# yemam3/SAC-RCBF

Measured on AMD Instinct MI355X. Metric: safe env steps/sec (dynamics+CBF-QP) at batch 65536, 1/2/4/8 MI355X, higher is better.
Workload: dtype f32 rows / f64 QP / f64 env

## Files before the change

### sac-rcbf_amd/csrc/rcbf_device.hpp

```cpp
#pragma once

#include <hip/hip_runtime.h>
#include <stdint.h>

#include "rcbf_hip.h"

namespace rcbf {

constexpr double kInf = __builtin_huge_val();


#ifdef RCBF_STUDY_QP_STAMPS
__device__ __forceinline__ void qp_stamp(int j) {
    __builtin_amdgcn_sched_barrier(0);
    unsigned long long t;
    asm volatile("s_memtime %0\n\ts_waitcnt lgkmcnt(0)" : "=s"(t)::"memory");
    __builtin_amdgcn_sched_barrier(0);
    if ((threadIdx.x & 63) == 0 && rcbf_qp_stamp_buf)
        rcbf_qp_stamp_buf[((int64_t)blockIdx.x * 4 + (threadIdx.x >> 6)) * 16 + j] = t;
}
__device__ __forceinline__ void qp_count(int j, bool f) {
    const unsigned long long n = __popcll(__ballot(f));
    if ((threadIdx.x & 63) == 0 && rcbf_qp_stamp_buf)
        rcbf_qp_stamp_buf[((int64_t)blockIdx.x * 4 + (threadIdx.x >> 6)) * 16 + j] = n;
// ... 1679 lines not shown
    double c, s;
    sincos(xs[2], &s, &c);
    double px = xs[0] + lp * c, py = xs[1] + lp * s;
    double g00 = c, g01 = -s * lp, g10 = s, g11 = c * lp;
    double mpx = mu[0] + lp * (-s) * mu[2], mpy = mu[1] + lp * c * mu[2];
    double spx = sig[0] + lp * (-s) * sig[2], spy = sig[1] + lp * c * sig[2];
    const double r2 = (1.2 * prm.hazards_radius) * (1.2 * prm.hazards_radius);
#pragma unroll
    for (int j = 0; j < K; ++j) {
        double dx = px - prm.hazards_xy[2 * j], dy = py - prm.hazards_xy[2 * j + 1];
        double hs = 0.5 * ((dx * dx + dy * dy) - r2);
        double a0 = dx * g00 + dy * g10, a1 = dx * g01 + dy * g11;
        G[j][0] = -a0;
        G[j][1] = -a1;
        G[j][2] = -1.0;
        h[j] = ((g * (hs * hs * hs) + (dx * mpx + dy * mpy)) + (a0 * u[0] + a1 * u[1])) -
               kd * (fabs(dx) * spx + fabs(dy) * spy);
    }
#pragma unroll
    for (int c2 = 0; c2 < 2; ++c2) {
        const int r0 = K + 2 * c2;
#pragma unroll
        for (int k = 0; k < 3; ++k) {
            G[r0][k] = (k == c2) ? 1.0 : 0.0;
            G[r0 + 1][k] = (k == c2) ? -1.0 : 0.0;
        }
        h[r0] = prm.u_max[c2] - u[c2];
        h[r0 + 1] = -prm.u_min[c2] + u[c2];
    }
}

struct CarsStepOut {
    float reward;
    double reward_d;
    double cost;
    bool done;
};

__device__ __forceinline__ double cars_env_pre(const rcbf_params& prm, double* xs, double& t, int& step,
                                               CarsStepOut& o) {
#pragma clang fp contract(off)
    const double kp = prm.kp, kb = prm.k_brake, dt = 0.02;
    double vdes0 = 30.0 - 10.0 * sin_small(0.2 * t);
    double acc[5];
    acc[0] = kp * (vdes0 - xs[1]);
#pragma unroll
    for (int i = 1; i < 5; ++i) acc[i] = kp * (30.0 - xs[2 * i + 1]);
    double d01 = xs[0] - xs[2], d12 = xs[2] - xs[4], d24 = xs[4] - xs[8];
    acc[1] += (-kb * d01) * (d01 < 6.0 ? 1.0 : 0.0);
    acc[2] += (-kb * d12) * (d12 < 6.0 ? 1.0 : 0.0);
    acc[4] += (-kb * d24) * (d24 < 13.0 ? 1.0 : 0.0);
#pragma unroll
    for (int i = 0; i < 5; ++i) acc[i] *= 1.1;
    double v[5];
#pragma unroll
    for (int i = 0; i < 5; ++i) v[i] = xs[2 * i + 1];
#pragma unroll
    for (int i = 0; i < 5; ++i) {
        xs[2 * i] += dt * v[i];
        if (i != 3) xs[2 * i + 1] += dt * acc[i];
    }
    t = t + dt;
    step += 1;
    o.done = step >= 300;
    double cost = 0.0;
    if (xs[4] - xs[6] < 2.99) cost -= 0.1;
    if (xs[6] - xs[8] < 2.99) cost -= 0.1;
    o.cost = cost;
    return acc[3];
}

template <typename A>
__device__ __forceinline__ void cars_env_post(double* xs, double acc3, A action, CarsStepOut& o) {
#pragma clang fp contract(off)
    const double dt = 0.02;
    const double gu = 50.0 * (double)action;
    xs[7] += dt * (acc3 + gu);
    A a2 = action * action;
    A r = (A)(-5.0) * (a2 < (A)0 ? -a2 : a2) / (A)300;
    o.reward = (float)r;
    o.reward_d = (double)r;
}

template <typename A>
__device__ __forceinline__ void cars_env_step(const rcbf_params& prm, double* xs, double& t, int& step, A action,
                                              CarsStepOut& o) {
    const double acc3 = cars_env_pre(prm, xs, t, step, o);
    cars_env_post<A>(xs, acc3, action, o);
}

__device__ __forceinline__ double div_const(double x, double d, double inv_d) {
    double q = x * inv_d;
    double r = fma(-q, d, x);
    return fma(r, inv_d, q);
}

__device__ __forceinline__ void cars_obs(const double* xs, double* o) {
#pragma unroll
    for (int i = 0; i < 5; ++i) {
        o[2 * i] = div_const(xs[2 * i], 100.0, 1.0 / 100.0);
        o[2 * i + 1] = div_const(xs[2 * i + 1], 30.0, 1.0 / 30.0);
    }
}

__device__ __forceinline__ void sincos_add_small(double c, double s, double d, double& c2, double& s2) {
    const double d2 = d * d;
    const double sd =
        d * fma(d2, fma(d2, fma(d2, fma(d2, 1.0 / 362880.0, -1.0 / 5040.0), 1.0 / 120.0), -1.0 / 6.0), 1.0);
    const double cd =
        fma(d2, fma(d2, fma(d2, fma(d2, 1.0 / 40320.0, -1.0 / 720.0), 1.0 / 24.0), -0.5), 1.0);
    c2 = fma(c, cd, -(s * sd));
    s2 = fma(s, cd, c * sd);
}

__device__ __forceinline__ double uni_goal_dist(const double* xs) {
#pragma clang fp contract(off)
    double d0 = 2.5 - xs[0], d1 = 2.5 - xs[1];
    return sqrt(d0 * d0 + d1 * d1);
}

__device__ __forceinline__ void uni_obs_cs(const double* xs, double c, double s, double gd, double* o) {
#pragma clang fp contract(off)
    double r0 = 2.5 - xs[0], r1 = 2.5 - xs[1];
    double v0 = r0 * c + r1 * s;
    double v1 = r0 * (-s) + r1 * c;
    double nrm = sqrt(v0 * v0 + v1 * v1) + 0.001;
    const double rn = rcp64_nz(nrm);
    o[0] = xs[0];
    o[1] = xs[1];
    o[2] = c;
    o[3] = s;
    o[4] = v0 * rn;
    o[5] = v1 * rn;
    o[6] = exp(-gd);
}

__device__ __forceinline__ void uni_obs(const double* xs, double* o) {
#pragma clang fp contract(off)
    double r0 = 2.5 - xs[0], r1 = 2.5 - xs[1];
    double gd = sqrt(r0 * r0 + r1 * r1);
    double c, s;
    sincos(xs[2], &s, &c);
    double v0 = r0 * c + r1 * s;
    double v1 = r0 * (-s) + r1 * c;
    double nrm = sqrt(v0 * v0 + v1 * v1) + 0.001;
    o[0] = xs[0];
    o[1] = xs[1];
    o[2] = c;
    o[3] = s;
    o[4] = v0 / nrm;
    o[5] = v1 / nrm;
    o[6] = exp(-gd);
}

struct UniStepOut {
    double reward;
    double cost;
    bool done;
    bool goal;
    double c, s, gd;
};

template <typename A, int KH = 0>
__device__ __forceinline__ void uni_env_step_cs(const rcbf_params& prm, double* xs, double& last_dist, int& step,
                                                const A* action, double c, double s, UniStepOut& o) {
#pragma clang fp contract(off)
    A a0c = action[0] < (A)(-1) ? (A)(-1) : (action[0] > (A)1 ? (A)1 : action[0]);
    A a1c = action[1] < (A)(-1) ? (A)(-1) : (action[1] > (A)1 ? (A)1 : action[1]);
    double a0 = (double)a0c, a1 = (double)a1c;
    const double dt = 0.02;
    xs[0] += dt * (c * a0);
    xs[1] += dt * (s * a0);
    const double th0 = xs[2];
    xs[2] += dt * a1;
    double c2, s2;
    sincos_add_small(c, s, xs[2] - th0, c2, s2);
    const double k = dt * 0.1;
    xs[0] -= (k * c2) * c2;
    xs[1] -= (k * s2) * c2;
    o.c = c2;
    o.s = s2;
    step += 1;
    double d = uni_goal_dist(xs);
    o.gd = d;
// ... 69 lines not shown
```

### sac-rcbf_amd/csrc/rcbf_safe_step.hpp

```cpp
#pragma once

#include <cstddef>

#include "rcbf_common.hpp"

#ifndef RCBF_KARG_PREFETCH
#define RCBF_KARG_PREFETCH 0
#endif
#ifndef RCBF_TRAJ_OBS_PLAIN
#define RCBF_TRAJ_OBS_PLAIN 0
#endif
#ifndef RCBF_EARLY_STORE
#define RCBF_EARLY_STORE 1
#endif
#ifndef RCBF_FUSED_CARRY
#define RCBF_FUSED_CARRY 1
#endif
#ifndef RCBF_FUSED_CARRY_SOLVE_FIRST
#define RCBF_FUSED_CARRY_SOLVE_FIRST 0
#endif

namespace rcbf {

template <int NL>
__device__ __forceinline__ void prefetch_kernargs() {
#if defined(__HIP_DEVICE_COMPILE__)
    __builtin_amdgcn_sched_barrier(0);
    const uint32_t* ka = (const uint32_t*)__builtin_amdgcn_kernarg_segment_ptr();
    uint32_t acc = 0;
#pragma unroll
    for (int l = 0; l < NL; ++l) acc ^= ka[16 * l];
    asm volatile("" ::"s"(acc));
    __builtin_amdgcn_sched_barrier(0);
#endif
}

template <int MODE>
__device__ __forceinline__ void load_state(const double* x, int64_t B, int64_t i, double* xs) {
    constexpr int NS = Dims<MODE, 1>::NS;
#pragma unroll
    for (int p = 0; p < NS / 2; ++p) {
        double2 v = ld_in2(&x[2 * (p * B + i)]);
        xs[2 * p] = v.x;
        xs[2 * p + 1] = v.y;
    }
    if constexpr (NS % 2) xs[NS - 1] = ld_in(&x[(NS - 1) * B + i]);
}

template <int MODE, typename XP = double*>
__device__ __forceinline__ void store_state(XP x, int64_t B, int64_t i, const double* xs) {
    constexpr int NS = Dims<MODE, 1>::NS;
#pragma unroll
    for (int p = 0; p < NS / 2; ++p) st_out2d(&x[2 * (p * B + i)], xs[2 * p], xs[2 * p + 1]);
    if constexpr (NS % 2) st_out(&x[(NS - 1) * B + i], xs[NS - 1]);
}

template <int MODE, bool WT = false, typename OP = float*>
__device__ __forceinline__ void store_obs32(OP obs, int64_t i, const double* xs,
                                            const double* obs_cache = nullptr) {
    constexpr int NO = Dims<MODE, 1>::NO;
    double o[NO];
    if constexpr (MODE == RCBF_MODE_UNICYCLE) {
        if (obs_cache && obs_cache[3] != 0.0)
            uni_obs_cs(xs, obs_cache[0], obs_cache[1], obs_cache[2], o);
        else
            env_obs<MODE>(xs, o);
    } else {
        env_obs<MODE>(xs, o);
    }
    if constexpr (MODE == RCBF_MODE_SIMULATED_CARS) {
        const OP ov = obs + i * NO;
#pragma unroll
        for (int k = 0; k < NO / 2; ++k) {
            if constexpr (WT) {
                const float pr[2] = {(float)o[2 * k], (float)o[2 * k + 1]};
                uint64_t w;
                __builtin_memcpy(&w, pr, 8);
                st_wt(reinterpret_cast<uint64_t*>(ov + 2 * k), w);
            } else {
                st_out2(ov + 2 * k, (float)o[2 * k], (float)o[2 * k + 1]);
            }
        }
    } else {
#pragma unroll
        for (int k = 0; k < NO; ++k) st_any<WT>(&obs[i * NO + k], (float)o[k]);
    }
}

template <int MODE, bool WT = false, bool SC1 = WT || MODE == RCBF_MODE_SIMULATED_CARS, typename OP = float*,
          bool PLAIN_ST = false, bool WHOLE = false>
__device__ __forceinline__ void store_obs_chunks(OP obs, int64_t base, const float* lds_wave, int lane) {
    constexpr int NO = Dims<MODE, 1>::NO;
    __builtin_amdgcn_wave_barrier();
    constexpr int CH = NO * 16;
    const float4* src = reinterpret_cast<const float4*>(lds_wave);
    const OP dst = obs + base * NO;
    constexpr int NJ = (CH + 63) / 64;
    float4 chunk[NJ];
    if constexpr (WHOLE) {
#pragma unroll
        for (int j = 0; j < NJ; ++j) {
            const int c = j * 64 + lane;
            chunk[j] = src[(j < CH / 64 || c < CH) ? c : lane];
        }
#pragma unroll
        for (int j = 0; j < NJ; ++j) asm volatile("" : "+v"(chunk[j].x), "+v"(chunk[j].y), "+v"(chunk[j].z), "+v"(chunk[j].w));
#pragma unroll
        for (int j = 0; j < NJ; ++j) {
            const int c = j * 64 + lane;
            if (j < CH / 64 || c < CH) {
                if constexpr (PLAIN_ST)
                    st_out4_plain(dst + 4 * c, chunk[j]);
                else
                    st_out4<SC1>(dst + 4 * c, chunk[j]);
            }
        }
        return;
    }
#pragma unroll
    for (int j = 0; j < NJ; ++j) {
        const int c = j * 64 + lane;
        if (CH % 64 == 0 || c < CH) chunk[j] = src[c];
    }
#pragma unroll
    for (int j = 0; j < NJ; ++j) {
        const int c = j * 64 + lane;
        if (CH % 64 == 0 || c < CH) {
            if constexpr (PLAIN_ST)
                st_out4_plain(dst + 4 * c, chunk[j]);
            else
                st_out4<SC1>(dst + 4 * c, chunk[j]);
        }
    }
}

template <int MODE, bool WT = false, bool SC1 = WT || MODE == RCBF_MODE_SIMULATED_CARS, typename OP = float*,
          bool PLAIN_ST = false>
__device__ __forceinline__ void store_obs32_staged(OP obs, int64_t i, int64_t B, const double* xs,
                                                   const double* obs_cache, float* lds_wave, int lane) {
    constexpr int NO = Dims<MODE, 1>::NO;
    const int64_t base = i - lane;
#ifdef RCBF_STUDY_EPW
    const bool full = blockDim.x != 64 && (base + 64 <= B) && ((reinterpret_cast<uintptr_t>(obs) & 15) == 0);
#else
    const bool full = (base + 64 <= B) && ((reinterpret_cast<uintptr_t>(obs) & 15) == 0);
#endif
    if (!full) {
        store_obs32<MODE, WT>(obs, i, xs, obs_cache);
        return;
    }
    double o[NO];
    if constexpr (MODE == RCBF_MODE_UNICYCLE) {
        if (obs_cache && obs_cache[3] != 0.0)
            uni_obs_cs(xs, obs_cache[0], obs_cache[1], obs_cache[2], o);
        else
            env_obs<MODE>(xs, o);
    } else {
        env_obs<MODE>(xs, o);
    }
    if constexpr (NO % 2 == 0) {
#pragma unroll
        for (int k = 0; k < NO / 2; ++k)
            *reinterpret_cast<float2*>(&lds_wave[lane * NO + 2 * k]) = make_float2((float)o[2 * k], (float)o[2 * k + 1]);
    } else {
#pragma unroll
        for (int k = 0; k < NO; ++k) lds_wave[lane * NO + k] = (float)o[k];
    }
    store_obs_chunks<MODE, WT, SC1, OP, PLAIN_ST>(obs, base, lds_wave, lane);
}

template <int MODE, typename OP>
__device__ __forceinline__ bool stage_obs32_row(OP obs, int64_t i, int64_t B, const float* o32, float* lds_wave,
                                                int lane) {
    constexpr int NO = Dims<MODE, 1>::NO;
    static_assert(NO % 2 == 0, "8-byte halves of a row");
    const int64_t base = i - lane;
#ifdef RCBF_STUDY_EPW
    const bool full_l = blockDim.x != 64 && (base + 64 <= B) && ((reinterpret_cast<uintptr_t>(obs) & 15) == 0);
#else
    const bool full_l = (base + 64 <= B) && ((reinterpret_cast<uintptr_t>(obs) & 15) == 0);
#endif
    const bool full = __builtin_amdgcn_readfirstlane((int)full_l) != 0;
    if (full) {
#pragma unroll
        for (int k = 0; k < NO / 2; ++k)
            *reinterpret_cast<float2*>(&lds_wave[lane * NO + 2 * k]) = make_float2(o32[2 * k], o32[2 * k + 1]);
    } else {
        const OP ov = obs + i * NO;
#pragma unroll
        for (int k = 0; k < NO / 2; ++k) st_out2(ov + 2 * k, o32[2 * k], o32[2 * k + 1]);
    }
    return full;
}

template <int SOLVER, int MODE, int K, bool ST, bool WT, bool GP = false,
          bool OBS_SC1 = WT || MODE == RCBF_MODE_SIMULATED_CARS, bool OBS_PLAIN = false, int CARRY = 0,
          bool TERM = false>
__device__ __forceinline__ void safe_step_body(
    const rcbf_params& prm, int64_t B, int64_t i, ptr_g<GP, double> __restrict__ x, ptr_g<GP, double> __restrict__ aux,
    ptr_g<GP, int32_t> __restrict__ step, ptr_g<GP, uint32_t> __restrict__ episode,
    ptr_g<GP, float> __restrict__ obs_out, ptr_g<GP, float> __restrict__ u_out, ptr_g<GP, float> __restrict__ reward,
    ptr_g<GP, float> __restrict__ cost, ptr_g<GP, uint8_t> __restrict__ done, ptr_g<GP, uint8_t> __restrict__ goal_met,
    ptr_g<GP, int32_t> __restrict__ status_out, ptr_g<GP, int32_t> fail_flag, int auto_reset,
    uint64_t seed, int64_t off, double* xs, double& a, int& st, const float* us, const float* m, const float* s,
    bool ep_pre, uint32_t ep0, const Stamps<ST>& stamps, float* obs_stage, char* wt_lds, int lane,
    bool* did_reset = nullptr, float* obs_c = nullptr, float (*G_c)[Dims<MODE, K>::N] = nullptr,
    float* h_c = nullptr, const float* u_nx = nullptr, ptr_g<GP, float> term_obs = nullptr) {
    using D = Dims<MODE, K>;
    static_assert(!TERM || (GP && !ST && !WT && SOLVER == RCBF_SOLVER_ACTIVE_SET &&
                            (MODE != RCBF_MODE_SIMULATED_CARS || RCBF_EARLY_STORE)),
                  "the terminal observation: the fused loop only");
    static_assert(CARRY == 0 || (MODE == RCBF_MODE_SIMULATED_CARS && RCBF_EARLY_STORE && !ST && !WT && GP &&
                                 SOLVER == RCBF_SOLVER_ACTIVE_SET && RCBF_FUSED_RAW_ROWS != 0),
                  "the carried observation: the cars fused loop only");
    const int64_t wbase = i - lane;
    const bool wfull = wbase + 64 <= B;
    constexpr int kWtBytes = WT ? 16 * 160 : 16;
    (void)wt_lds;
    (void)wfull;
    (void)kWtBytes;
    float rew, cst;
    bool dn, gm;
    int status;
    float uf[D::NU];
    double oc[4] = {0.0, 0.0, 0.0, 0.0};
    if constexpr (MODE == RCBF_MODE_SIMULATED_CARS && RCBF_EARLY_STORE && !ST) {
        float s32[D::NS];
        if constexpr (CARRY == 0) state_from_env<MODE>(xs, s32);
        if constexpr (CARRY == 1) state_from_obs32<MODE>(obs_c, s32);
        constexpr bool kRowsFirst = SOLVER == RCBF_SOLVER_ACTIVE_SET && RCBF_FUSED_RAW_ROWS != 0;
        LayerState<MODE, K> L;
        if constexpr (CARRY == 2) {
#pragma unroll
            for (int r = 0; r < D::M; ++r) {
                L.h[r] = h_c[r];
#pragma unroll
                for (int k = 0; k < D::N; ++k) L.G[r][k] = G_c[r][k];
            }
        } else if constexpr (kRowsFirst) {
            diff_rows<MODE, K>(prm, s32, us, m, s, L.G, L.h, nullptr);
        }
        constexpr bool kSolveFirst = CARRY == 2 && RCBF_FUSED_CARRY_SOLVE_FIRST != 0;
        if constexpr (kSolveFirst) {
            layer_solve_raw<MODE, K>(prm, us, uf, L);
            __builtin_amdgcn_sched_barrier(0);
        }
        CarsStepOut o;
        const double acc3 = cars_env_pre(prm, xs, a, st, o);
        dn = o.done;
        cst = (float)o.cost;
        gm = false;
        const bool rs = auto_reset && dn;
        if (rs) {
            if constexpr (TERM) {
                double ot[D::NO];
                env_obs<MODE>(xs, ot);
#pragma unroll
                for (int k = 0; k < D::NO; ++k)
                    if (k != 7) st_out(&term_obs[i * D::NO + k], (float)ot[k]);
                oc[0] = xs[7];
            }
            const uint32_t ep = episode ? (ep_pre ? ep0 : episode[i]) + 1u : 0u;
            if (episode) {
                if constexpr (WT)
                    st_wt(&episode[i], ep);
                else
                    episode[i] = ep;
            }
            env_reset_one<MODE>(nullptr, i, seed, off, ep, xs, a, st);
        }
#pragma unroll
        for (int p = 0; p < D::NS / 2; ++p)
            if (p != 3) st_any2d<WT>(&x[2 * (p * B + i)], xs[2 * p], xs[2 * p + 1]);
        if constexpr (WT) {
            using E = WtStage<8, 4>;
            char* const dst[2] = {reinterpret_cast<char*>(aux + wbase), reinterpret_cast<char*>(step + wbase)};
            const uint64_t val[2] = {wt_bits(a), wt_bits(st)};
            E::store(wt_lds, lane, wfull, dst, val);
        } else {
            st_out(&aux[i], a);
            st_out(&step[i], st);
        }
        __builtin_amdgcn_sched_barrier(0);
        if constexpr (kSolveFirst) {
        } else if constexpr (kRowsFirst) {
            layer_solve_raw<MODE, K>(prm, us, uf, L);
        } else {
            layer_forward<SOLVER, MODE, K, false, false, RCBF_FUSED_RAW_ROWS != 0>(prm, s32, us, m, s, uf, L);
        }
        status = L.qp.status;
        const double v3_reset = xs[7];
        if constexpr (TERM) xs[7] = rs ? oc[0] : xs[7];
        cars_env_post<float>(xs, acc3, uf[0], o);
        if constexpr (TERM) {
            if (rs) st_out(&term_obs[i * D::NO + 7], (float)div_const(xs[7], 30.0, 1.0 / 30.0));
        }
        xs[7] = rs ? v3_reset : xs[7];
        rew = o.reward;
        st_any2d<WT>(&x[2 * (3 * B + i)], xs[6], xs[7]);
    } else {
        if constexpr (TERM) {
            static_assert(MODE == RCBF_MODE_UNICYCLE, "the cars loop takes the early-store path");
            safe_step_one<SOLVER, MODE, K, ST, WT>(prm, i, xs, a, st, episode, us, m, s, uf, rew, cst, dn, gm, status,
                                                   0, seed, off, stamps, oc, ep_pre, ep0);
            if (auto_reset && dn) {
                double ot[D::NO];
                uni_obs_cs(xs, oc[0], oc[1], oc[2], ot);
#pragma unroll
                for (int k = 0; k < D::NO; ++k) st_out(&term_obs[i * D::NO + k], (float)ot[k]);
                const uint32_t ep = episode ? (ep_pre ? ep0 : episode[i]) + 1u : 0u;
                if (episode) episode[i] = ep;
                env_reset_one<MODE>(nullptr, i, seed, off, ep, xs, a, st);
                oc[0] = 1.0;
                oc[1] = 0.0;
                oc[2] = a;
                oc[3] = 1.0;
            }
        } else {
            safe_step_one<SOLVER, MODE, K, ST, WT>(prm, i, xs, a, st, episode, us, m, s, uf, rew, cst, dn, gm, status,
                                                   auto_reset, seed, off, stamps, oc, ep_pre, ep0);
        }
        if constexpr (WT) {
#pragma unroll
            for (int p = 0; p < D::NS / 2; ++p) st_wt2d(&x[2 * (p * B + i)], xs[2 * p], xs[2 * p + 1]);
        } else {
            store_state<MODE>(x, B, i, xs);
            st_out(&aux[i], a);
            st_out(&step[i], st);
        }
    }
    bool obs_staged = false;
    if constexpr (CARRY != 0) {
        double o[D::NO];
        env_obs<MODE>(xs, o);
#pragma unroll
        for (int k = 0; k < D::NO; ++k) obs_c[k] = (float)o[k];
        obs_staged = stage_obs32_row<MODE>(obs_out, i, B, obs_c, obs_stage, lane);
        if constexpr (CARRY == 2) {
            float s32n[D::NS];
            state_from_obs32<MODE>(obs_c, s32n);
            diff_rows<MODE, K>(prm, s32n, u_nx, m, s, G_c, h_c, nullptr);
            asm volatile("" : "+v"(G_c[0][0]), "+v"(G_c[1][0]), "+v"(h_c[0]), "+v"(h_c[1]), "+v"(h_c[2]), "+v"(h_c[3]));
        }
    } else {
        store_obs32_staged<MODE, WT, OBS_SC1, ptr_g<GP, float>, OBS_PLAIN>(obs_out, i, B, xs, oc, obs_stage, lane);
    }
    if constexpr (WT) {
        constexpr int NU4 = 4 * D::NU;
        float ufc[D::NU];
#pragma unroll
        for (int c = 0; c < D::NU; ++c) ufc[c] = uf[c];
        char* const u_d = reinterpret_cast<char*>(u_out + wbase * D::NU);
        char* const r_d = reinterpret_cast<char*>(reward + wbase);
        char* const c_d = reinterpret_cast<char*>(cost + wbase);
        char* const d_d = reinterpret_cast<char*>(done + wbase);
        uint64_t u_v = 0;
        __builtin_memcpy(&u_v, ufc, sizeof(ufc));
        const uint64_t r_v = wt_bits(rew), c_v = wt_bits(cst), d_v = (uint64_t)dn;
        if constexpr (MODE == RCBF_MODE_SIMULATED_CARS && RCBF_EARLY_STORE) {
            if (goal_met) {
                using E = WtStage<NU4, 4, 4, 1, 1>;
                char* const dst[5] = {u_d, r_d, c_d, d_d, reinterpret_cast<char*>(goal_met + wbase)};
                const uint64_t val[5] = {u_v, r_v, c_v, d_v, (uint64_t)gm};
                E::store(wt_lds, lane, wfull, dst, val);
            } else {
                using E = WtStage<NU4, 4, 4, 1>;
                char* const dst[4] = {u_d, r_d, c_d, d_d};
                const uint64_t val[4] = {u_v, r_v, c_v, d_v};
                E::store(wt_lds, lane, wfull, dst, val);
            }
        } else {
            static_assert(D::NS % 2 == 1, "the late write-through block carries the odd state component");
            char* const x_d = reinterpret_cast<char*>(x + (D::NS - 1) * B + wbase);
            char* const a_d = reinterpret_cast<char*>(aux + wbase);
            char* const s_d = reinterpret_cast<char*>(step + wbase);
            const uint64_t x_v = wt_bits(xs[D::NS - 1]), a_v = wt_bits(a), s_v = wt_bits(st);
            if (goal_met) {
                using E = WtStage<8, 8, 4, NU4, 4, 4, 1, 1>;
                static_assert(E::kBytes <= kWtBytes, "wt_lds");
                char* const dst[8] = {x_d, a_d, s_d, u_d, r_d, c_d, d_d, reinterpret_cast<char*>(goal_met + wbase)};
                const uint64_t val[8] = {x_v, a_v, s_v, u_v, r_v, c_v, d_v, (uint64_t)gm};
                E::store(wt_lds, lane, wfull, dst, val);
            } else {
                using E = WtStage<8, 8, 4, NU4, 4, 4, 1>;
                char* const dst[7] = {x_d, a_d, s_d, u_d, r_d, c_d, d_d};
                const uint64_t val[7] = {x_v, a_v, s_v, u_v, r_v, c_v, d_v};
                E::store(wt_lds, lane, wfull, dst, val);
            }
        }
    } else {
#pragma unroll
        for (int c = 0; c < D::NU; ++c) st_out(&u_out[i * D::NU + c], uf[c]);
        st_out(&reward[i], rew);
        st_out(&cost[i], cst);
        st_out(&done[i], (uint8_t)dn);
        if (goal_met) st_out(&goal_met[i], (uint8_t)gm);
    }
    if constexpr (CARRY != 0) {
        if (obs_staged)
            store_obs_chunks<MODE, WT, OBS_SC1, ptr_g<GP, float>, OBS_PLAIN, true>(obs_out, wbase, obs_stage, lane);
    }
    if (did_reset) *did_reset = auto_reset && dn;
    stamps.mark(6, false);
    if constexpr (WT) {
        if (status_out) st_wt(&status_out[i], (int32_t)status);
        if (status != RCBF_QP_OK && fail_flag) atomicOr(fail_flag, 1 << status);
        asm volatile("s_waitcnt vmcnt(0)" ::: "memory");
    } else {
        report(status, status_out, i, fail_flag);
    }
}

template <int SOLVER, int MODE, int K, bool ST = false, int BS = kBlock, bool SPAN = false>
__global__ void __launch_bounds__(BS) k_safe_step(int64_t B, double* __restrict__ x, double* __restrict__ aux,
                                                      int32_t* __restrict__ step, const float* __restrict__ u_rl,
                                                      uint32_t* __restrict__ episode, const float* __restrict__ mu,
                                                      const float* __restrict__ sigma, float* __restrict__ obs_out,
                                                      float* __restrict__ u_out, float* __restrict__ reward,
                                                      float* __restrict__ cost, uint8_t* __restrict__ done,
                                                      uint8_t* __restrict__ goal_met,
                                                      int32_t* __restrict__ status_out, int32_t* fail_flag,
                                                      int auto_reset, uint64_t seed, int64_t off, rcbf_params prm,
                                                      int prior_cols = 0, unsigned long long* stamp_buf = nullptr) {
    using D = Dims<MODE, K>;
    constexpr bool WT = RCBF_WT_OUT != 0 && !ST;
    int64_t i = env_index<BS>();
    if (i >= B) return;
    constexpr int kWtBytes = WT ? 16 * 160 : 16;
    __shared__ __attribute__((aligned(16))) char wt_lds_all[BS / 64][kWtBytes];
    char* wt_lds = wt_lds_all[threadIdx.x >> 6];
    unsigned long long span_t0 = 0, span_c0 = 0;
    if constexpr (SPAN) {
        span_t0 = __builtin_amdgcn_s_memrealtime();
        span_c0 = __builtin_amdgcn_s_memtime();
    }
    Stamps<ST> stamps;
    stamps.buf = stamp_buf;
    stamps.mark(0, false);
    double xs[D::NS];
    load_state<MODE>(x, B, i, xs);
    double a = ld_in(&aux[i]);
    int st = ld_in(&step[i]);
    float us[D::NU], m[D::NS], s[D::NS];
#pragma unroll
    for (int c = 0; c < D::NU; ++c) us[c] = ld_in(&u_rl[i * D::NU + c]);
#if RCBF_KARG_PREFETCH
    prefetch_kernargs<RCBF_KARG_PREFETCH>();
#else
    if constexpr (MODE == RCBF_MODE_SIMULATED_CARS) prefetch_kernargs<7>();
#endif
    const bool ep_pre = episode && reset_foreseeable<MODE>(st, a);
    uint32_t ep0 = 0;
    if (ep_pre) ep0 = episode[i];
    if (prior_cols) {
#pragma unroll
        for (int k = 0; k < D::NS; ++k) {
            m[k] = 0.0f;
            s[k] = prior_sigma<MODE>(k);
        }
        if constexpr (MODE == RCBF_MODE_SIMULATED_CARS) {
            if (sigma) {
                s[5] = ld_in(&sigma[i]);
                s[7] = ld_in(&sigma[B + i]);
                s[9] = ld_in(&sigma[2 * B + i]);
            }
        } else {
#pragma unroll
            for (int k = 0; k < D::NS; ++k) {
                if (mu) m[k] = ld_in(&mu[k * B + i]);
                if (sigma) s[k] = ld_in(&sigma[k * B + i]);
            }
        }
    } else {
#pragma unroll
        for (int k = 0; k < D::NS; ++k) {
            m[k] = mu ? mu[i * D::NS + k] : 0.0f;
            s[k] = sigma ? sigma[i * D::NS + k] : prior_sigma<MODE>(k);
        }
    }
    stamps.mark(1, true);
    __shared__ float obs_stage[BS / 64][64 * D::NO];
    safe_step_body<SOLVER, MODE, K, ST, WT>(prm, B, i, x, aux, step, episode, obs_out, u_out, reward, cost, done,
                                            goal_met, status_out, fail_flag, auto_reset, seed, off, xs, a, st, us, m,
                                            s, ep_pre, ep0, stamps, obs_stage[threadIdx.x >> 6], wt_lds,
                                            threadIdx.x & 63);
    stamps.mark(7, true);
    if constexpr (SPAN) {
        asm volatile("s_waitcnt vmcnt(0)" ::: "memory");
        const unsigned long long t1 = __builtin_amdgcn_s_memrealtime();
        const unsigned long long c1 = __builtin_amdgcn_s_memtime();
        if ((threadIdx.x & 63) == 0) {
            const int64_t w = ((int64_t)blockIdx.x * BS + threadIdx.x) >> 6;
            typedef unsigned long long u2 __attribute__((ext_vector_type(2)));
            *reinterpret_cast<u2*>(stamp_buf + 4 * w) = u2{span_t0, t1};
            *reinterpret_cast<u2*>(stamp_buf + 4 * w + 2) = u2{span_c0, c1};
        }
    }
}

template <int MODE>
constexpr int fused_carry() {
    return MODE == RCBF_MODE_SIMULATED_CARS ? RCBF_FUSED_CARRY : 0;
}

template <int MODE, int K, bool TRAJ = false>
constexpr bool fused_plain() {
    return !TRAJ && (MODE == RCBF_MODE_SIMULATED_CARS || K == 1);
}

struct SafeStepsArgs {
    int64_t B;
    double* x;
    double* aux;
    int32_t* step;
    const float* const* u_tab;
    uint32_t* episode;
    const float* mu;
    const float* sigma;
    float* obs_out;
    float* u_out;
    float* reward;
    float* cost;
    uint8_t* done;
    uint8_t* goal_met;
    int32_t* status_out;
    int32_t* fail_flag;
    int32_t auto_reset;
    uint64_t seed;
    int64_t off;
    rcbf_params prm;
    int32_t prior_cols;
    int32_t n_u;
    int32_t steps;
    int32_t ju0;
};
static_assert(offsetof(SafeStepsArgs, auto_reset) == 128 && offsetof(SafeStepsArgs, seed) == 136 &&
                  offsetof(SafeStepsArgs, prm) == 152 && offsetof(SafeStepsArgs, prior_cols) == 392 &&
                  offsetof(SafeStepsArgs, n_u) == 396 && offsetof(SafeStepsArgs, steps) == 400 &&
                  offsetof(SafeStepsArgs, ju0) == 404 && sizeof(SafeStepsArgs) == 408,
              "kernarg layout");

struct SafeStepsTrajArgs {
    SafeStepsArgs s;
    int32_t traj_mask;
    int64_t traj_pitch;
};
static_assert(offsetof(SafeStepsTrajArgs, traj_mask) == 408 && offsetof(SafeStepsTrajArgs, traj_pitch) == 416 &&
                  sizeof(SafeStepsTrajArgs) == 424,
              "kernarg layout");

struct TrajTail {
    int64_t pitch;
    int32_t mask;
    int32_t pad;
};

__device__ __forceinline__ TrajTail traj_from_kernargs(uint32_t off) {
    TrajTail t{0, 0, 0};
#if defined(__HIP_DEVICE_COMPILE__)
    typedef const char __attribute__((address_space(4)))* cbytes_t;
    const cbytes_t ka = (cbytes_t)__builtin_amdgcn_kernarg_segment_ptr() + off;
    t.mask = *reinterpret_cast<const int32_t __attribute__((address_space(4)))*>(
        ka + offsetof(SafeStepsTrajArgs, traj_mask));
    t.pitch = *reinterpret_cast<const int64_t __attribute__((address_space(4)))*>(
        ka + offsetof(SafeStepsTrajArgs, traj_pitch));
#endif
    return t;
}

template <int BS>
__device__ __forceinline__ TrajTail* traj_stage_of(int wave) {
    __shared__ TrajTail stage[BS / 64];
    return &stage[wave];
}

struct SafeStepsTermArgs {
    SafeStepsTrajArgs t;
    float* term_obs;
};
static_assert(offsetof(SafeStepsTermArgs, term_obs) == 424 && sizeof(SafeStepsTermArgs) == 432, "kernarg layout");

__device__ __forceinline__ gptr<float> term_from_kernargs() {
    uint64_t p = 0;
#if defined(__HIP_DEVICE_COMPILE__)
    typedef const char __attribute__((address_space(4)))* cbytes_t;
    const cbytes_t ka = (cbytes_t)__builtin_amdgcn_kernarg_segment_ptr();
    p = *reinterpret_cast<const uint64_t __attribute__((address_space(4)))*>(
        ka + offsetof(SafeStepsTermArgs, term_obs));
#endif
    return reinterpret_cast<gptr<float>>(p);
}

template <int MODE, int K, int BS = kBlock>
__global__ void __launch_bounds__(BS) k_safe_steps(int64_t B, double* __restrict__ x, double* __restrict__ aux,
                                                       int32_t* __restrict__ step,
                                                       const float* const* __restrict__ u_tab,
                                                       uint32_t* __restrict__ episode, const float* __restrict__ mu,
                                                       const float* __restrict__ sigma, float* __restrict__ obs_out,
                                                       float* __restrict__ u_out, float* __restrict__ reward,
                                                       float* __restrict__ cost, uint8_t* __restrict__ done,
                                                       uint8_t* __restrict__ goal_met,
                                                       int32_t* __restrict__ status_out, int32_t* fail_flag,
                                                       int auto_reset, uint64_t seed, int64_t off, rcbf_params prm,
                                                       int prior_cols, int n_u, int steps, int ju0) {
    constexpr bool TRAJ = false;
#define RCBF_LOOP_TERM 0
#include "rcbf_safe_steps_loop.inc"
#undef RCBF_LOOP_TERM
}

template <int MODE, int K, int BS = kBlock>
__global__ void __launch_bounds__(BS) k_safe_steps_traj(
    int64_t B, double* __restrict__ x, double* __restrict__ aux, int32_t* __restrict__ step,
    const float* const* __restrict__ u_tab, uint32_t* __restrict__ episode, const float* __restrict__ mu,
    const float* __restrict__ sigma, float* __restrict__ obs_out, float* __restrict__ u_out,
    float* __restrict__ reward, float* __restrict__ cost, uint8_t* __restrict__ done, uint8_t* __restrict__ goal_met,
    int32_t* __restrict__ status_out, int32_t* fail_flag, int auto_reset, uint64_t seed, int64_t off, rcbf_params prm,
    int prior_cols, int n_u, int steps, int ju0, int32_t traj_mask, int64_t traj_pitch) {
    (void)traj_mask;
    (void)traj_pitch;
    constexpr bool TRAJ = true;
#define RCBF_LOOP_TERM 0
#include "rcbf_safe_steps_loop.inc"
#undef RCBF_LOOP_TERM
}

template <int MODE, int K, int BS = kBlock>
__global__ void __launch_bounds__(BS) k_safe_steps_term(
    int64_t B, double* __restrict__ x, double* __restrict__ aux, int32_t* __restrict__ step,
    const float* const* __restrict__ u_tab, uint32_t* __restrict__ episode, const float* __restrict__ mu,
    const float* __restrict__ sigma, float* __restrict__ obs_out, float* __restrict__ u_out,
    float* __restrict__ reward, float* __restrict__ cost, uint8_t* __restrict__ done, uint8_t* __restrict__ goal_met,
    int32_t* __restrict__ status_out, int32_t* fail_flag, int auto_reset, uint64_t seed, int64_t off, rcbf_params prm,
    int prior_cols, int n_u, int steps, int ju0, int32_t traj_mask, int64_t traj_pitch, float* __restrict__ term_obs) {
    (void)traj_mask;
    (void)traj_pitch;
    (void)term_obs;
    constexpr bool TRAJ = true;
#define RCBF_LOOP_TERM 1
#include "rcbf_safe_steps_loop.inc"
#undef RCBF_LOOP_TERM
}

#define RCBF_SAFE_STEPS_INSTANTIATE_BS(MODE_, K_, BS_)                                                              \
    template __global__ void k_safe_steps<MODE_, K_, BS_>(                                                          \
        int64_t, double* __restrict__, double* __restrict__, int32_t* __restrict__, const float* const* __restrict__, \
        uint32_t* __restrict__, const float* __restrict__, const float* __restrict__, float* __restrict__,          \
        float* __restrict__, float* __restrict__, float* __restrict__, uint8_t* __restrict__, uint8_t* __restrict__, \
        int32_t* __restrict__, int32_t*, int, uint64_t, int64_t, rcbf_params, int, int, int, int)
#define RCBF_SAFE_STEPS_INSTANTIATE(MODE_, K_)      \
    RCBF_SAFE_STEPS_INSTANTIATE_BS(MODE_, K_, 64);  \
    RCBF_SAFE_STEPS_INSTANTIATE_BS(MODE_, K_, 128); \
    RCBF_SAFE_STEPS_INSTANTIATE_BS(MODE_, K_, 256)

#define RCBF_SAFE_STEPS_TRAJ_INSTANTIATE_BS(MODE_, K_, BS_)                                                         \
    template __global__ void k_safe_steps_traj<MODE_, K_, BS_>(                                                     \
        int64_t, double* __restrict__, double* __restrict__, int32_t* __restrict__, const float* const* __restrict__, \
        uint32_t* __restrict__, const float* __restrict__, const float* __restrict__, float* __restrict__,          \
        float* __restrict__, float* __restrict__, float* __restrict__, uint8_t* __restrict__, uint8_t* __restrict__, \
        int32_t* __restrict__, int32_t*, int, uint64_t, int64_t, rcbf_params, int, int, int, int, int32_t, int64_t)
#define RCBF_SAFE_STEPS_TRAJ_INSTANTIATE(MODE_, K_)      \
    RCBF_SAFE_STEPS_TRAJ_INSTANTIATE_BS(MODE_, K_, 64);  \
    RCBF_SAFE_STEPS_TRAJ_INSTANTIATE_BS(MODE_, K_, 128); \
    RCBF_SAFE_STEPS_TRAJ_INSTANTIATE_BS(MODE_, K_, 256)

#define RCBF_SAFE_STEPS_TERM_INSTANTIATE_BS(MODE_, K_, BS_)                                                         \
    template __global__ void k_safe_steps_term<MODE_, K_, BS_>(                                                     \
        int64_t, double* __restrict__, double* __restrict__, int32_t* __restrict__, const float* const* __restrict__, \
        uint32_t* __restrict__, const float* __restrict__, const float* __restrict__, float* __restrict__,          \
        float* __restrict__, float* __restrict__, float* __restrict__, uint8_t* __restrict__, uint8_t* __restrict__, \
        int32_t* __restrict__, int32_t*, int, uint64_t, int64_t, rcbf_params, int, int, int, int, int32_t, int64_t, \
        float* __restrict__)
#define RCBF_SAFE_STEPS_TERM_INSTANTIATE(MODE_, K_)      \
    RCBF_SAFE_STEPS_TERM_INSTANTIATE_BS(MODE_, K_, 64);  \
    RCBF_SAFE_STEPS_TERM_INSTANTIATE_BS(MODE_, K_, 128); \
    RCBF_SAFE_STEPS_TERM_INSTANTIATE_BS(MODE_, K_, 256)

}
```

### sac-rcbf_amd/csrc/rcbf_safe_steps_loop.inc

```
    using D = Dims<MODE, K>;
    constexpr int SOLVER = RCBF_SOLVER_ACTIVE_SET;
    constexpr bool WT = false;
    constexpr bool PLAIN = fused_plain<MODE, K, TRAJ>();
    constexpr bool OBS_SC1 = false;
    int64_t i = env_index<BS>();
    if (i >= B) return;
    double xs[D::NS];
    load_state<MODE>(x, B, i, xs);
    double a = ld_in(&aux[i]);
    int st = ld_in(&step[i]);
    typedef const uint64_t __attribute__((address_space(4)))* ctab_t;
    const ctab_t tab = (ctab_t)reinterpret_cast<const uint64_t*>(u_tab);
    float us[D::NU], m[D::NS], s[D::NS];
    {
        const gptr<const float> u0 = reinterpret_cast<gptr<const float>>(tab[ju0]);
#pragma unroll
        for (int c = 0; c < D::NU; ++c) us[c] = ld_in(&u0[i * D::NU + c]);
    }
    uint32_t epr = episode ? ld_in(&episode[i]) : 0u;
    int ju = ju0 + 1 == n_u ? 0 : ju0 + 1;
    gptr<const float> u_next = reinterpret_cast<gptr<const float>>(tab[ju]);
    if constexpr (MODE == RCBF_MODE_SIMULATED_CARS) prefetch_kernargs<7>();
    if (prior_cols) {
#pragma unroll
        for (int k = 0; k < D::NS; ++k) {
            m[k] = 0.0f;
            s[k] = prior_sigma<MODE>(k);
        }
        if constexpr (MODE == RCBF_MODE_SIMULATED_CARS) {
            if (sigma) {
                s[5] = ld_in(&sigma[i]);
                s[7] = ld_in(&sigma[B + i]);
                s[9] = ld_in(&sigma[2 * B + i]);
            }
        } else {
#pragma unroll
            for (int k = 0; k < D::NS; ++k) {
                if (mu) m[k] = ld_in(&mu[k * B + i]);
                if (sigma) s[k] = ld_in(&sigma[k * B + i]);
            }
        }
    } else {
#pragma unroll
        for (int k = 0; k < D::NS; ++k) {
            m[k] = mu ? mu[i * D::NS + k] : 0.0f;
            s[k] = sigma ? sigma[i * D::NS + k] : prior_sigma<MODE>(k);
        }
    }
    __shared__ float obs_stage[BS / 64][64 * D::NO];
    __shared__ rcbf_params prm_stage[K >= 8 ? BS / 64 : 1];
    if constexpr (K >= 8) {
        prm_stage[threadIdx.x >> 6] = prm;
        if constexpr (TRAJ) *traj_stage_of<BS>(threadIdx.x >> 6) = traj_from_kernargs(0);
        __builtin_amdgcn_wave_barrier();
    }
    const Stamps<false> stamps{};
    int64_t Bv = B;
    gptr<double> xv = (gptr<double>)x;
    gptr<double> auxv = (gptr<double>)aux;
    gptr<int32_t> stepv = (gptr<int32_t>)step;
    gptr<uint32_t> epv = (gptr<uint32_t>)episode;
    gptr<float> obsv = (gptr<float>)obs_out;
    gptr<float> uv = (gptr<float>)u_out;
    gptr<float> rewv = (gptr<float>)reward;
    gptr<float> costv = (gptr<float>)cost;
    gptr<uint8_t> donev = (gptr<uint8_t>)done;
    gptr<uint8_t> goalv = (gptr<uint8_t>)goal_met;
    gptr<int32_t> statv = (gptr<int32_t>)status_out;
    gptr<int32_t> failv = (gptr<int32_t>)fail_flag;
    uint64_t tabv = reinterpret_cast<uint64_t>(u_tab), unextv = reinterpret_cast<uint64_t>(u_next);
    int arv = auto_reset, lanev = threadIdx.x & 63, nuv = n_u, juv = ju, leftv = steps,
        widv = threadIdx.x >> 6;
    uint64_t seedv = seed;
    int64_t offv = off;
#define RCBF_OPAQUE_V()                                                                                          \
    if constexpr (!PLAIN) {                                                                                      \
        asm volatile("" : "+a"(xv), "+a"(auxv), "+a"(stepv), "+a"(epv), "+a"(obsv), "+a"(uv), "+a"(rewv));     \
        asm volatile("" : "+a"(costv), "+a"(donev), "+a"(goalv), "+a"(statv), "+a"(failv), "+a"(epr),         \
                     "+a"(Bv), "+a"(arv), "+a"(lanev), "+a"(i));                                                 \
        asm volatile("" : "+a"(widv), "+a"(tabv), "+a"(nuv), "+a"(juv), "+a"(leftv), "+a"(seedv), "+a"(offv),   \
                     "+a"(unextv));                                                                              \
    }
    RCBF_OPAQUE_V();
#if RCBF_LOOP_TERM
    static_assert(TRAJ && !PLAIN, "k_safe_steps_term: a trajectory kernel");
    gptr<float> termv = term_from_kernargs();
    asm volatile("" : "+a"(termv));
#endif
    __builtin_amdgcn_s_waitcnt(0x0f70);
    constexpr int CARRY = fused_carry<MODE>();
    float obs_c[D::NO], Gc[D::M][D::N], hc[D::M];
    if constexpr (CARRY != 0) {
        double o[D::NO];
        env_obs<MODE>(xs, o);
#pragma unroll
        for (int k = 0; k < D::NO; ++k) obs_c[k] = (float)o[k];
        if constexpr (CARRY == 2) {
            float s32[D::NS];
            state_from_obs32<MODE>(obs_c, s32);
            diff_rows<MODE, K>(prm, s32, us, m, s, Gc, hc, nullptr);
        }
    }
#pragma nounroll
    while (leftv > 0) {
        RCBF_OPAQUE_V();
#if RCBF_LOOP_TERM
        asm volatile("" : "+a"(termv));
#endif
        if constexpr (PLAIN && CARRY != 0) asm volatile("" : "+v"(epv), "+v"(failv));
        const rcbf_params* prm_p = &prm;
        if constexpr (!PLAIN) {
#pragma unroll
            for (int k = 0; k < D::NS; ++k) asm volatile("" : "+a"(m[k]), "+a"(s[k]));
            if constexpr (K >= 8) {
                uint32_t prm_voff = 0;
                asm volatile("" : "+v"(prm_voff));
                prm_p = reinterpret_cast<const rcbf_params*>(reinterpret_cast<const char*>(&prm_stage[widv]) +
                                                             prm_voff);
            } else {
                uint32_t prm_off = 0;
                asm volatile("" : "+s"(prm_off));
                prm_p = reinterpret_cast<const rcbf_params*>(reinterpret_cast<const char*>(&prm) + prm_off);
            }
        }
        const rcbf_params& prm_j = *prm_p;
        float un[D::NU];
#pragma unroll
        for (int c = 0; c < D::NU; ++c) un[c] = 0.0f;
        --leftv;
        if (leftv > 0) {
            const gptr<const float> u1 = reinterpret_cast<gptr<const float>>(unextv);
#pragma unroll
            for (int c = 0; c < D::NU; ++c) un[c] = ld_in(&u1[i * D::NU + c]);
        }
        uint64_t unext2;
        {
            int nu_s = n_u, ju_s = juv;
            uint64_t tab_s = reinterpret_cast<uint64_t>(u_tab);
            if constexpr (!PLAIN) {
                tab_s = ((uint64_t)(uint32_t)__builtin_amdgcn_readfirstlane((int)(tabv >> 32)) << 32) |
                        (uint32_t)__builtin_amdgcn_readfirstlane((int)(uint32_t)tabv);
                nu_s = __builtin_amdgcn_readfirstlane(nuv);
                ju_s = __builtin_amdgcn_readfirstlane(juv);
            }
            ju_s = ju_s + 1 == nu_s ? 0 : ju_s + 1;
            juv = ju_s;
            unext2 = reinterpret_cast<ctab_t>(tab_s)[ju_s];
        }
        bool rs = false;
        constexpr bool OBS_PLAIN = TRAJ && RCBF_TRAJ_OBS_PLAIN != 0;
#if RCBF_LOOP_TERM
        safe_step_body<SOLVER, MODE, K, false, WT, true, OBS_SC1, OBS_PLAIN, CARRY, true>(
            prm_j, Bv, i, xv, auxv, stepv, epv, obsv, uv, rewv, costv, donev, goalv, statv, failv, arv, seedv, offv, xs,
            a, st, us, m, s, epv != nullptr, epr, stamps, obs_stage[widv], nullptr, lanev, &rs, CARRY ? obs_c : nullptr,
            CARRY ? Gc : nullptr, CARRY ? hc : nullptr, CARRY ? un : nullptr, termv);
#else
        safe_step_body<SOLVER, MODE, K, false, WT, true, OBS_SC1, OBS_PLAIN, CARRY>(
            prm_j, Bv, i, xv, auxv, stepv, epv, obsv, uv, rewv, costv, donev, goalv, statv, failv, arv, seedv, offv, xs,
            a, st, us, m, s, epv != nullptr, epr, stamps, obs_stage[widv], nullptr, lanev, &rs, CARRY ? obs_c : nullptr, CARRY ? Gc : nullptr, CARRY ? hc : nullptr,
            CARRY ? un : nullptr);
#endif
        epr += rs ? 1u : 0u;
        __builtin_amdgcn_wave_barrier();
        asm volatile("" ::: "memory");
        if constexpr (TRAJ) {
            TrajTail t;
            if constexpr (!PLAIN && K >= 8) {
                uint32_t voff = 0;
                asm volatile("" : "+v"(voff));
                t = *reinterpret_cast<const TrajTail*>(reinterpret_cast<const char*>(traj_stage_of<BS>(widv)) + voff);
            } else {
                uint32_t soff = 0;
                if constexpr (!PLAIN) asm volatile("" : "+s"(soff));
                t = traj_from_kernargs(soff);
            }
            const int64_t row = t.pitch;
            obsv += (t.mask & RCBF_TRAJ_OBS) ? row * D::NO : (int64_t)0;
            uv += (t.mask & RCBF_TRAJ_U) ? row * D::NU : (int64_t)0;
            rewv += (t.mask & RCBF_TRAJ_REWARD) ? row : (int64_t)0;
            costv += (t.mask & RCBF_TRAJ_COST) ? row : (int64_t)0;
            donev += (t.mask & RCBF_TRAJ_DONE) ? row : (int64_t)0;
            goalv += (t.mask & RCBF_TRAJ_GOAL_MET) ? row : (int64_t)0;
            statv += (t.mask & RCBF_TRAJ_STATUS) ? row : (int64_t)0;
#if RCBF_LOOP_TERM
            termv += (t.mask & RCBF_TRAJ_TERM_OBS) ? row * D::NO : (int64_t)0;
#endif
        }
#pragma unroll
        for (int c = 0; c < D::NU; ++c) us[c] = un[c];
        if constexpr (!PLAIN) asm volatile("" : "+s"(unext2));
        unextv = unext2;
    }
#undef RCBF_OPAQUE_V
```

Before: 53.83 billion.

## Add lean fused cars step with hoisted full-check, cheaper division, early LDS obs loads

Adds a LEAN variant of the fused cars safe-step body for the non-trajectory multi-step kernel, enabled by default (all four bits set). The wave-uniform full-tile check for obs staging is hoisted out of the step loop. Reward division by 300 becomes a guarded FMA-refined reciprocal. The obs constants are negated and pinned in registers. The LDS obs chunks are now loaded before the scalar output stores, with reward and cost computed afterwards, so LDS latency overlaps the global stores. This targets per-step instruction count and LDS wait stalls, at the cost of more live vector registers and tighter scheduling barriers.

Result: faster. 54.59 billion (median of 6 runs) (+1.4%).

```diff
diff --git a/sac-rcbf_amd/csrc/rcbf_device.hpp b/sac-rcbf_amd/csrc/rcbf_device.hpp
--- a/sac-rcbf_amd/csrc/rcbf_device.hpp
+++ b/sac-rcbf_amd/csrc/rcbf_device.hpp
@@ -1785,6 +1785,42 @@
     o.reward_d = (double)r;
 }
 
+constexpr uint32_t kDiv300GuardLo = 0x9f800000u;
+constexpr uint32_t kDiv300GuardHi = 0xf1800000u;
+__device__ __forceinline__ float div300_f32(float x) {
+#pragma clang fp contract(off)
+    constexpr float c = 1.0f / 300.0f;
+    const float q = x * c;
+    const float r = __builtin_fmaf(-q, 300.0f, x);
+    float res = __builtin_fmaf(r, c, q);
+    if (__builtin_expect(__builtin_bit_cast(uint32_t, x) - kDiv300GuardLo >= kDiv300GuardHi - kDiv300GuardLo, 0))
+        res = x / 300.0f;
+    return res;
+}
+
+template <bool DIV = true>
+__device__ __forceinline__ float cars_reward_lean(float action) {
+#pragma clang fp contract(off)
+    const float a2 = action * action;
+    const float x = -5.0f * (a2 < 0.0f ? -a2 : a2);
+    if constexpr (DIV)
+        return div300_f32(x);
+    else
+        return x / 300.0f;
+}
+
+template <bool REWARD>
+__device__ __forceinline__ void cars_env_post_lean(double* xs, double acc3, float action, CarsStepOut& o) {
+#pragma clang fp contract(off)
+    const double dt = 0.02;
+    const double gu = 50.0 * (double)action;
+    xs[7] += dt * (acc3 + gu);
+    if constexpr (REWARD) {
+        o.reward = cars_reward_lean(action);
+        o.reward_d = (double)o.reward;
+    }
+}
+
 template <typename A>
 __device__ __forceinline__ void cars_env_step(const rcbf_params& prm, double* xs, double& t, int& step, A action,
                                               CarsStepOut& o) {
@@ -1803,6 +1839,20 @@
     for (int i = 0; i < 5; ++i) {
         o[2 * i] = div_const(xs[2 * i], 100.0, 1.0 / 100.0);
         o[2 * i + 1] = div_const(xs[2 * i + 1], 30.0, 1.0 / 30.0);
+    }
+}
+
+__device__ __forceinline__ double div_const_negd(double x, double neg_d, double inv_d) {
+    double q = x * inv_d;
+    double r = fma(q, neg_d, x);
+    return fma(r, inv_d, q);
+}
+
+__device__ __forceinline__ void cars_obs_lean(const double* xs, double* o, double n100, double n30) {
+#pragma unroll
+    for (int i = 0; i < 5; ++i) {
+        o[2 * i] = div_const_negd(xs[2 * i], n100, 1.0 / 100.0);
+        o[2 * i + 1] = div_const_negd(xs[2 * i + 1], n30, 1.0 / 30.0);
     }
 }
 
diff --git a/sac-rcbf_amd/csrc/rcbf_safe_step.hpp b/sac-rcbf_amd/csrc/rcbf_safe_step.hpp
--- a/sac-rcbf_amd/csrc/rcbf_safe_step.hpp
+++ b/sac-rcbf_amd/csrc/rcbf_safe_step.hpp
@@ -19,6 +19,13 @@
 #ifndef RCBF_FUSED_CARRY_SOLVE_FIRST
 #define RCBF_FUSED_CARRY_SOLVE_FIRST 0
 #endif
+#ifndef RCBF_FUSED_LEAN
+#define RCBF_FUSED_LEAN 15
+#endif
+#define RCBF_LEAN_DIV 1
+#define RCBF_LEAN_LDS 2
+#define RCBF_LEAN_FULL 4
+#define RCBF_LEAN_COPIES 8
 
 namespace rcbf {
 
@@ -134,6 +141,44 @@
     }
 }
 
+template <int MODE>
+constexpr int obs_chunks_per_lane() {
+    return (Dims<MODE, 1>::NO * 16 + 63) / 64;
+}
+
+typedef float obs_chunk_t __attribute__((ext_vector_type(4)));
+
+template <int MODE>
+__device__ __forceinline__ void load_obs_chunks(const float* lds_wave, int lane, obs_chunk_t* chunk) {
+    constexpr int CH = Dims<MODE, 1>::NO * 16, NJ = obs_chunks_per_lane<MODE>();
+    __builtin_amdgcn_wave_barrier();
+    const obs_chunk_t* src = reinterpret_cast<const obs_chunk_t*>(lds_wave);
+#pragma unroll
+    for (int j = 0; j < NJ; ++j) {
+        const int c = j * 64 + lane;
+        chunk[j] = src[(j < CH / 64 || c < CH) ? c : lane];
+    }
+}
+
+template <int MODE, bool SC1, typename OP, bool PLAIN_ST>
+__device__ __forceinline__ void store_obs_chunks_loaded(OP obs, int64_t base, int lane, obs_chunk_t* chunk) {
+    constexpr int NO = Dims<MODE, 1>::NO, CH = NO * 16, NJ = obs_chunks_per_lane<MODE>();
+    const OP dst = obs + base * NO;
+#pragma unroll
+    for (int j = 0; j < NJ; ++j) asm volatile("" : "+v"(chunk[j]));
+#pragma unroll
+    for (int j = 0; j < NJ; ++j) {
+        const int c = j * 64 + lane;
+        if (j < CH / 64 || c < CH) {
+            const float4 v = make_float4(chunk[j].x, chunk[j].y, chunk[j].z, chunk[j].w);
+            if constexpr (PLAIN_ST)
+                st_out4_plain(dst + 4 * c, v);
+            else
+                st_out4<SC1>(dst + 4 * c, v);
+        }
+    }
+}
+
 template <int MODE, bool WT = false, bool SC1 = WT || MODE == RCBF_MODE_SIMULATED_CARS, typename OP = float*,
           bool PLAIN_ST = false>
 __device__ __forceinline__ void store_obs32_staged(OP obs, int64_t i, int64_t B, const double* xs,
@@ -171,7 +216,7 @@
 
 template <int MODE, typename OP>
 __device__ __forceinline__ bool stage_obs32_row(OP obs, int64_t i, int64_t B, const float* o32, float* lds_wave,
-                                                int lane) {
+                                                int lane, int obs_full = -1) {
     constexpr int NO = Dims<MODE, 1>::NO;
     static_assert(NO % 2 == 0, "8-byte halves of a row");
     const int64_t base = i - lane;
@@ -180,7 +225,7 @@
 #else
     const bool full_l = (base + 64 <= B) && ((reinterpret_cast<uintptr_t>(obs) & 15) == 0);
 #endif
-    const bool full = __builtin_amdgcn_readfirstlane((int)full_l) != 0;
+    const bool full = obs_full >= 0 ? obs_full != 0 : __builtin_amdgcn_readfirstlane((int)full_l) != 0;
     if (full) {
 #pragma unroll
         for (int k = 0; k < NO / 2; ++k)
@@ -195,7 +240,7 @@
 
 template <int SOLVER, int MODE, int K, bool ST, bool WT, bool GP = false,
           bool OBS_SC1 = WT || MODE == RCBF_MODE_SIMULATED_CARS, bool OBS_PLAIN = false, int CARRY = 0,
-          bool TERM = false>
+          bool TERM = false, int LEAN = 0>
 __device__ __forceinline__ void safe_step_body(
     const rcbf_params& prm, int64_t B, int64_t i, ptr_g<GP, double> __restrict__ x, ptr_g<GP, double> __restrict__ aux,
     ptr_g<GP, int32_t> __restrict__ step, ptr_g<GP, uint32_t> __restrict__ episode,
@@ -205,8 +250,12 @@
     uint64_t seed, int64_t off, double* xs, double& a, int& st, const float* us, const float* m, const float* s,
     bool ep_pre, uint32_t ep0, const Stamps<ST>& stamps, float* obs_stage, char* wt_lds, int lane,
     bool* did_reset = nullptr, float* obs_c = nullptr, float (*G_c)[Dims<MODE, K>::N] = nullptr,
-    float* h_c = nullptr, const float* u_nx = nullptr, ptr_g<GP, float> term_obs = nullptr) {
+    float* h_c = nullptr, const float* u_nx = nullptr, ptr_g<GP, float> term_obs = nullptr, int obs_full = -1,
+    const double* obs_negd = nullptr) {
     using D = Dims<MODE, K>;
+    static_assert(LEAN == 0 || (CARRY != 0 && !TERM), "the lean step: the cars k_safe_steps kernels only");
+    (void)obs_full;
+    (void)obs_negd;
     static_assert(!TERM || (GP && !ST && !WT && SOLVER == RCBF_SOLVER_ACTIVE_SET &&
                             (MODE != RCBF_MODE_SIMULATED_CARS || RCBF_EARLY_STORE)),
                   "the terminal observation: the fused loop only");
@@ -220,6 +269,8 @@
     (void)wfull;
     (void)kWtBytes;
     float rew, cst;
+    double cost_d = 0.0;
+    (void)cost_d;
     bool dn, gm;
     int status;
     float uf[D::NU];
@@ -248,7 +299,8 @@
         CarsStepOut o;
         const double acc3 = cars_env_pre(prm, xs, a, st, o);
         dn = o.done;
-        cst = (float)o.cost;
+        if constexpr ((LEAN & RCBF_LEAN_LDS) == 0) cst = (float)o.cost;
+        cost_d = o.cost;
         gm = false;
         const bool rs = auto_reset && dn;
         if (rs) {
@@ -291,12 +343,17 @@
         status = L.qp.status;
         const double v3_reset = xs[7];
         if constexpr (TERM) xs[7] = rs ? oc[0] : xs[7];
-        cars_env_post<float>(xs, acc3, uf[0], o);
+        if constexpr ((LEAN & RCBF_LEAN_LDS) != 0)
+            cars_env_post_lean<false>(xs, acc3, uf[0], o);
+        else if constexpr ((LEAN & RCBF_LEAN_DIV) != 0)
+            cars_env_post_lean<true>(xs, acc3, uf[0], o);
+        else
+            cars_env_post<float>(xs, acc3, uf[0], o);
         if constexpr (TERM) {
             if (rs) st_out(&term_obs[i * D::NO + 7], (float)div_const(xs[7], 30.0, 1.0 / 30.0));
         }
         xs[7] = rs ? v3_reset : xs[7];
-        rew = o.reward;
+        if constexpr ((LEAN & RCBF_LEAN_LDS) == 0) rew = o.reward;
         st_any2d<WT>(&x[2 * (3 * B + i)], xs[6], xs[7]);
     } else {
         if constexpr (TERM) {
@@ -332,10 +389,16 @@
     bool obs_staged = false;
     if constexpr (CARRY != 0) {
         double o[D::NO];
-        env_obs<MODE>(xs, o);
+        if constexpr ((LEAN & RCBF_LEAN_COPIES) != 0)
+            cars_obs_lean(xs, o, obs_negd[0], obs_negd[1]);
+        else
+            env_obs<MODE>(xs, o);
 #pragma unroll
         for (int k = 0; k < D::NO; ++k) obs_c[k] = (float)o[k];
-        obs_staged = stage_obs32_row<MODE>(obs_out, i, B, obs_c, obs_stage, lane);
+        if constexpr ((LEAN & RCBF_LEAN_FULL) != 0)
+            obs_staged = stage_obs32_row<MODE>(obs_out, i, B, obs_c, obs_stage, lane, obs_full);
+        else
+            obs_staged = stage_obs32_row<MODE>(obs_out, i, B, obs_c, obs_stage, lane);
         if constexpr (CARRY == 2) {
             float s32n[D::NS];
             state_from_obs32<MODE>(obs_c, s32n);
@@ -388,15 +451,31 @@
                 E::store(wt_lds, lane, wfull, dst, val);
             }
         }
-    } else {
+    } else if constexpr ((LEAN & RCBF_LEAN_LDS) != 0) {
+        obs_chunk_t chunk[obs_chunks_per_lane<MODE>()];
+        load_obs_chunks<MODE>(obs_stage, lane, chunk);
+        __builtin_amdgcn_sched_barrier(0);
+        float ua = uf[0];
+        asm volatile("" : "+v"(ua), "+v"(cost_d));
+        rew = cars_reward_lean<(LEAN & RCBF_LEAN_DIV) != 0>(ua);
+        cst = (float)cost_d;
 #pragma unroll
         for (int c = 0; c < D::NU; ++c) st_out(&u_out[i * D::NU + c], uf[c]);
         st_out(&reward[i], rew);
         st_out(&cost[i], cst);
         st_out(&done[i], (uint8_t)dn);
         if (goal_met) st_out(&goal_met[i], (uint8_t)gm);
-    }
-    if constexpr (CARRY != 0) {
+        __builtin_amdgcn_sched_barrier(0);
+        if (obs_staged) store_obs_chunks_loaded<MODE, OBS_SC1, ptr_g<GP, float>, OBS_PLAIN>(obs_out, wbase, lane, chunk);
+    } else {
+#pragma unroll
+        for (int c = 0; c < D::NU; ++c) st_out(&u_out[i * D::NU + c], uf[c]);
+        st_out(&reward[i], rew);
+        st_out(&cost[i], cst);
+        st_out(&done[i], (uint8_t)dn);
+        if (goal_met) st_out(&goal_met[i], (uint8_t)gm);
+    }
+    if constexpr (CARRY != 0 && (LEAN & RCBF_LEAN_LDS) == 0) {
         if (obs_staged)
             store_obs_chunks<MODE, WT, OBS_SC1, ptr_g<GP, float>, OBS_PLAIN, true>(obs_out, wbase, obs_stage, lane);
     }
@@ -501,6 +580,11 @@
 template <int MODE>
 constexpr int fused_carry() {
     return MODE == RCBF_MODE_SIMULATED_CARS ? RCBF_FUSED_CARRY : 0;
+}
+
+template <int MODE, bool TRAJ>
+constexpr int fused_lean() {
+    return MODE == RCBF_MODE_SIMULATED_CARS && !TRAJ && fused_carry<MODE>() != 0 ? RCBF_FUSED_LEAN : 0;
 }
 
 template <int MODE, int K, bool TRAJ = false>
@@ -604,9 +688,11 @@
                                                        int auto_reset, uint64_t seed, int64_t off, rcbf_params prm,
                                                        int prior_cols, int n_u, int steps, int ju0) {
     constexpr bool TRAJ = false;
+#define RCBF_LOOP_TRAJ 0
 #define RCBF_LOOP_TERM 0
 #include "rcbf_safe_steps_loop.inc"
 #undef RCBF_LOOP_TERM
+#undef RCBF_LOOP_TRAJ
 }
 
 template <int MODE, int K, int BS = kBlock>
@@ -620,9 +706,11 @@
     (void)traj_mask;
     (void)traj_pitch;
     constexpr bool TRAJ = true;
+#define RCBF_LOOP_TRAJ 1
 #define RCBF_LOOP_TERM 0
 #include "rcbf_safe_steps_loop.inc"
 #undef RCBF_LOOP_TERM
+#undef RCBF_LOOP_TRAJ
 }
 
 template <int MODE, int K, int BS = kBlock>
@@ -637,9 +725,11 @@
     (void)traj_pitch;
     (void)term_obs;
     constexpr bool TRAJ = true;
+#define RCBF_LOOP_TRAJ 1
 #define RCBF_LOOP_TERM 1
 #include "rcbf_safe_steps_loop.inc"
 #undef RCBF_LOOP_TERM
+#undef RCBF_LOOP_TRAJ
 }
 
 #define RCBF_SAFE_STEPS_INSTANTIATE_BS(MODE_, K_, BS_)                                                              \
diff --git a/sac-rcbf_amd/csrc/rcbf_safe_steps_loop.inc b/sac-rcbf_amd/csrc/rcbf_safe_steps_loop.inc
--- a/sac-rcbf_amd/csrc/rcbf_safe_steps_loop.inc
+++ b/sac-rcbf_amd/csrc/rcbf_safe_steps_loop.inc
@@ -89,6 +89,15 @@
 #endif
     __builtin_amdgcn_s_waitcnt(0x0f70);
     constexpr int CARRY = fused_carry<MODE>();
+#if !RCBF_LOOP_TRAJ
+    constexpr int LEAN = fused_lean<MODE, TRAJ>();
+    double obs_negd[2] = {-100.0, -30.0};
+    if constexpr ((LEAN & RCBF_LEAN_COPIES) != 0) asm volatile("" : "+v"(obs_negd[0]), "+v"(obs_negd[1]));
+    int obs_fullv = -1;
+    if constexpr ((LEAN & RCBF_LEAN_FULL) != 0)
+        obs_fullv = __builtin_amdgcn_readfirstlane(
+            (int)((i - lanev + 64 <= B) && ((reinterpret_cast<uintptr_t>(obs_out) & 15) == 0)));
+#endif
     float obs_c[D::NO], Gc[D::M][D::N], hc[D::M];
     if constexpr (CARRY != 0) {
         double o[D::NO];
@@ -154,11 +163,16 @@
             prm_j, Bv, i, xv, auxv, stepv, epv, obsv, uv, rewv, costv, donev, goalv, statv, failv, arv, seedv, offv, xs,
             a, st, us, m, s, epv != nullptr, epr, stamps, obs_stage[widv], nullptr, lanev, &rs, CARRY ? obs_c : nullptr,
             CARRY ? Gc : nullptr, CARRY ? hc : nullptr, CARRY ? un : nullptr, termv);
-#else
+#elif RCBF_LOOP_TRAJ
         safe_step_body<SOLVER, MODE, K, false, WT, true, OBS_SC1, OBS_PLAIN, CARRY>(
             prm_j, Bv, i, xv, auxv, stepv, epv, obsv, uv, rewv, costv, donev, goalv, statv, failv, arv, seedv, offv, xs,
             a, st, us, m, s, epv != nullptr, epr, stamps, obs_stage[widv], nullptr, lanev, &rs, CARRY ? obs_c : nullptr, CARRY ? Gc : nullptr, CARRY ? hc : nullptr,
             CARRY ? un : nullptr);
+#else
+        safe_step_body<SOLVER, MODE, K, false, WT, true, OBS_SC1, OBS_PLAIN, CARRY, false, LEAN>(
+            prm_j, Bv, i, xv, auxv, stepv, epv, obsv, uv, rewv, costv, donev, goalv, statv, failv, arv, seedv, offv, xs,
+            a, st, us, m, s, epv != nullptr, epr, stamps, obs_stage[widv], nullptr, lanev, &rs, CARRY ? obs_c : nullptr, CARRY ? Gc : nullptr, CARRY ? hc : nullptr,
+            CARRY ? un : nullptr, nullptr, obs_fullv, obs_negd);
 #endif
         epr += rs ? 1u : 0u;
         __builtin_amdgcn_wave_barrier();
```
